# preacherwhite/Deformable-3D-Gaussians

Hardware: AMD Instinct MI355X
Metric: train iters/s (deform+raster fwd+bwd), 100k Gaussians @ 800x800 (higher is better)
Workload: dtype fp32

## Files before the change

### deformable-3d-gaussians_amd/csrc/mlp_split.hip

```cpp
#include <hip/hip_runtime.h>

#include <atomic>
#include <cassert>

#include <algorithm>
#include <cmath>
#include <cstdlib>
#include <map>
#include <mutex>
#include <type_traits>
#include <vector>

#include "dgs_common.h"
#include "mlp_shared.h"

namespace dgs {
namespace mlps {

using namespace mlpc;

typedef float f32x16 __attribute__((ext_vector_type(16)));
typedef float f32x4 __attribute__((ext_vector_type(4)));
typedef float f32x2 __attribute__((ext_vector_type(2)));
typedef _Float16 h16x8 __attribute__((ext_vector_type(8)));
// ... 78 lines not shown
}

__device__ __forceinline__ void lds_fmax(uint32_t *p, float v) {
    __hip_atomic_fetch_max(p, __float_as_uint(v), __ATOMIC_RELAXED, __HIP_MEMORY_SCOPE_WORKGROUP);
}

struct alignas(16) ScaleLDS {
    float ksc[12][4];
    float amax[2][16][4];
    float ain[2][4];
    uint32_t bsync[8][4];
    uint32_t bmax[10];
    uint32_t wstat[10];
};
constexpr int BS_XE = 0, BS_TE = 1, BS_TIN = 2, BS_TH = 3, BS_TET = 4, BS_G = 5, BS_GTE = 6;

__device__ inline float4 amax_of4(const ScaleLDS *sc, int par, int nw) {
    float4 m = make_float4(0.f, 0.f, 0.f, 0.f);
    for (int w = 0; w < nw; w++) {
        const float4 v = *reinterpret_cast<const float4 *>(sc->amax[par][w]);
        m = make_float4(fmaxf(m.x, v.x), fmaxf(m.y, v.y), fmaxf(m.z, v.z), fmaxf(m.w, v.w));
    }
    return m;
}
__device__ __forceinline__ float f4get(const float4 &v, int q) { return q == 0 ? v.x : q == 1 ? v.y : q == 2 ? v.z : v.w; }

#define MF16(a, b, c) __builtin_amdgcn_mfma_f32_16x16x32_f16((a), (b), (c), 0, 0, 0)

struct AFrag {
    h16x8 h, l;
};

__device__ inline AFrag load_a(const h16x8 *p) { return AFrag{p[0], p[64]}; }

__device__ inline AFrag load_b(const h16x8 *p, int q) { return AFrag{p[16 * q], p[BM + 16 * q]}; }

__device__ inline f32x4 zero4() { return f32x4{0.f, 0.f, 0.f, 0.f}; }

__device__ inline void mma3(const AFrag &a, const AFrag &b, f32x4 &acc, f32x4 &lo) {
    lo = MF16(a.l, b.h, lo);
    lo = MF16(a.h, b.l, lo);
    acc = MF16(a.h, b.h, acc);
}

__device__ __forceinline__ float a_inv(const h16x8 *tile_slot0) {
    return reinterpret_cast<const float *>(tile_slot0 + 128)[0];
}

#ifdef DGS_MLP_PROFILE
__device__ unsigned long long *dgs_mlps_prof;
#define DGS_STAMP(k)                                                                                   \
    do {                                                                                               \
        if (threadIdx.x == 0 && p0 == (int)blockIdx.x * BM)                                            \
            dgs_mlps_prof[blockIdx.x * 64 + (k)] = __builtin_amdgcn_s_memtime();                       \
    } while (0)
#define DGS_WSTAMP(k, L)                                                                               \
    do {                                                                                               \
        if (L == 3 && (threadIdx.x & 63) == 0 && p0 == (int)blockIdx.x * BM)                           \
            dgs_mlps_prof[blockIdx.x * 64 + (k) + (threadIdx.x >> 6)] = __builtin_amdgcn_s_memtime();  \
    } while (0)
#ifndef DGS_PROF_LAYER
#define DGS_PROF_LAYER 3
#endif
#define DGS_WSTAMP8(k, L)                                                                              \
    do {                                                                                               \
        if (L == DGS_PROF_LAYER && (threadIdx.x & 63) == 0 && p0 == (int)blockIdx.x * BM)              \
            dgs_mlps_prof[blockIdx.x * 64 + (k) + (threadIdx.x >> 6)] = __builtin_amdgcn_s_memtime();  \
    } while (0)
#else
#define DGS_WSTAMP8(k, L) \
    do {                  \
    } while (0)
#define DGS_WSTAMP(k, L) \
    do {                 \
    } while (0)
#define DGS_STAMP(k) \
    do {             \
    } while (0)
#endif

struct NoPre {
    __device__ void operator()() const {}
};

__device__ uint32_t dgs_mlps_guard_expired;

#ifdef DGS_CLOCK_STAMPS
constexpr int CLK_BLOCKS = 2048;
__device__ unsigned long long dgs_clk[3][CLK_BLOCKS][6];
struct ClkStamp {
    unsigned long long t, r;
    __device__ ClkStamp() : t(__builtin_amdgcn_s_memtime()), r(__builtin_amdgcn_s_memrealtime()) {}
    __device__ void end(int k) const {
        const unsigned long long t1 = __builtin_amdgcn_s_memtime(), r1 = __builtin_amdgcn_s_memrealtime();
        if (threadIdx.x == 0 && blockIdx.x < CLK_BLOCKS) {
            unsigned long long *p = dgs_clk[k][blockIdx.x];
            p[0] = t; p[1] = t1; p[2] = r; p[3] = r1;
            p[4] = (unsigned long long)__builtin_amdgcn_s_getreg((31 << 11) | 4) |
                   ((unsigned long long)__builtin_amdgcn_s_getreg((31 << 11) | 20) << 32);
        }
    }
};
#define CLK_BEGIN() const ClkStamp clk_
#define CLK_END(k) clk_.end(k)
#else
#define CLK_BEGIN()
#define CLK_END(k)
#endif
#ifndef DGS_SPIN_SLEEP
#define DGS_SPIN_SLEEP 1
#endif
__device__ __forceinline__ uint32_t lds_peek(const uint32_t *f) {
    return __hip_atomic_load(f, __ATOMIC_RELAXED, __HIP_MEMORY_SCOPE_WORKGROUP);
}
__device__ __forceinline__ void lds_wait_ge(const uint32_t *f, uint32_t target, uint32_t seen) {
    if (__builtin_amdgcn_readfirstlane(seen) < target) {
        int guard = 0;
#pragma clang loop unroll(disable)
        do {
            __builtin_amdgcn_s_sleep(DGS_SPIN_SLEEP);
            seen = lds_peek(f);
        } while (__builtin_amdgcn_readfirstlane(seen) < target && ++guard < (1 << 20));
        if (guard == (1 << 20) && (threadIdx.x & 63) == 0)
            __hip_atomic_fetch_add(&dgs_mlps_guard_expired, 1u, __ATOMIC_RELAXED, __HIP_MEMORY_SCOPE_AGENT);
    }
    asm volatile("" ::: "memory");
}
__device__ __forceinline__ void lds_signal(uint32_t *f, int lane) {
    asm volatile("" ::: "memory");
    if (lane == 0) __hip_atomic_fetch_add(f, 1u, __ATOMIC_RELAXED, __HIP_MEMORY_SCOPE_WORKGROUP);
}

struct NoGate {
    __device__ uint32_t peek(int) const { return 0; }
    __device__ void need(int, uint32_t) const {}
    __device__ void done(int) const {}
};

struct HGate {
    uint32_t *wr, *rd;
    int k0;
    uint32_t wt;
    bool sig;
    int lane;
    __device__ uint32_t peek(int k) const { return k < k0 ? 0xffffffffu : lds_peek(wr + (k - k0)); }
    __device__ void need(int k, uint32_t seen) const {
        if (k >= k0) lds_wait_ge(wr + (k - k0), wt, seen);
    }
    __device__ void done(int k) const {
        if (sig && k >= k0) lds_signal(rd + (k - k0), lane);
    }
};

template <int NK, int NQ_, class Pre = NoPre, class Gate = NoGate, int SKIP = (1 << 20), unsigned BND = 0u>
__device__ inline void gemm(const h16x8 *__restrict__ Aw, const h16x8 *lds, int g0, int q0, int lane,
                            f32x4 (&acc)[NQ_], float (&ib)[NQ_], const float (*ksc)[4], Pre pre = Pre(),
                            Gate gate = Gate()) {
    static_assert(NK >= 1, "empty GEMM");
    const int kq = lane >> 4, col = lane & 15;
    const h16x8 *Ap = Aw + lane;
    const int bunit = (g0 + kq) * UG + 16 * q0 + col;
    constexpr int AK = KSLOT;
    constexpr int BK = KG * UG;
    auto bofs = [](int k) { return (k + (k >= SKIP ? 1 : 0)) * BK; };
    auto kidx = [&](int k) { return (g0 >> 2) + k + (k >= SKIP ? 1 : 0); };
    auto kbase = [&](int k) {
        int u = bunit + bofs(k);
        asm volatile("" : "+v"(u));
        return lds + u;
    };
    constexpr int RING = 2;
    AFrag ring[RING];
#pragma unroll
    for (int k = 0; k < RING; k++)
        if (k < NK) ring[k] = load_a(Ap + k * AK);
    pre();
    gate.need(0, gate.peek(0));
    float cur[NQ_], nxt[NQ_];
#pragma unroll
    for (int q = 0; q < NQ_; q++) nxt[q] = cur[q] = ksc[kidx(0)][q0 + q];
    const h16x8 *Bk = kbase(0);
    AFrag b = load_b(Bk, 0);
    f32x4 lo[NQ_];
#pragma unroll
    for (int q = 0; q < NQ_; q++) lo[q] = zero4();
#pragma unroll
    for (int k = 0; k < NK; k++) {
        __builtin_amdgcn_sched_barrier(0);
        if (k > 0) gate.done(k - 1);
        if (k > 0 && k < 32 && ((BND >> k) & 1u)) {
#pragma unroll
            for (int q = 0; q < NQ_; q++) {
                acc[q] = (acc[q] + lo[q]) * (cur[q] / nxt[q]);
                lo[q] = zero4();
                cur[q] = nxt[q];
            }
        }
        const uint32_t seen = k + 1 < NK ? gate.peek(k + 1) : 0u;
#pragma unroll
        for (int q = 0; q < NQ_; q++) {
            AFrag nb;
            if (q + 1 < NQ_) nb = load_b(Bk, q + 1);
            else if (k + 1 < NK) {
                gate.need(k + 1, seen);
                if (k + 1 < 32 && ((BND >> (k + 1)) & 1u))
#pragma unroll
                    for (int q2 = 0; q2 < NQ_; q2++) nxt[q2] = ksc[kidx(k + 1)][q0 + q2];
                Bk = kbase(k + 1);
                nb = load_b(Bk, 0);
            }
            __builtin_amdgcn_sched_barrier(0);
            mma3(ring[k % RING], b, acc[q], lo[q]);
            if (q + 1 < NQ_ || k + 1 < NK) b = nb;
            __builtin_amdgcn_sched_barrier(0);
        }
        if (k + RING < NK) ring[k % RING] = load_a(Ap + (k + RING) * AK);
        __builtin_amdgcn_sched_barrier(0);
    }
    gate.done(NK - 1);
#pragma unroll
    for (int q = 0; q < NQ_; q++) {
        acc[q] += lo[q];
        ib[q] = cur[q];
    }
}

template <int NK, int NQ_, class Pre = NoPre, class Gate = NoGate, int SKIP = (1 << 20), unsigned BND = 0u>
__device__ inline void gemm2(const h16x8 *__restrict__ Aw, int astride, const h16x8 *lds, int g0, int q0, int lane,
                             f32x4 (&acc)[2][NQ_], float (&ib)[NQ_], const float (*ksc)[4], Pre pre = Pre(),
                             Gate gate = Gate()) {
    static_assert(NK >= 1, "empty GEMM");
    const int kq = lane >> 4, col = lane & 15;
    const h16x8 *Ap0 = Aw + lane, *Ap1 = Aw + astride + lane;
    const int bunit = (g0 + kq) * UG + 16 * q0 + col;
    constexpr int AK = KSLOT;
    constexpr int BK = KG * UG;
    auto bofs = [](int k) { return (k + (k >= SKIP ? 1 : 0)) * BK; };
    auto kidx = [&](int k) { return (g0 >> 2) + k + (k >= SKIP ? 1 : 0); };
    auto kbase = [&](int k) {
        int u = bunit + bofs(k);
        asm volatile("" : "+v"(u));
        return lds + u;
    };
    constexpr int RING = 2;
    AFrag ring[RING][2];
#pragma unroll
    for (int k = 0; k < RING; k++)
        if (k < NK) {
            ring[k][0] = load_a(Ap0 + k * AK);
            ring[k][1] = load_a(Ap1 + k * AK);
        }
    pre();
    gate.need(0, gate.peek(0));
    float cur[NQ_], nxt[NQ_];
#pragma unroll
    for (int q = 0; q < NQ_; q++) nxt[q] = cur[q] = ksc[kidx(0)][q0 + q];
    const h16x8 *Bk = kbase(0);
    AFrag b = load_b(Bk, 0);
    f32x4 lo[2][NQ_];
#pragma unroll
    for (int t = 0; t < 2; t++)
#pragma unroll
        for (int q = 0; q < NQ_; q++) lo[t][q] = zero4();
#pragma unroll
    for (int k = 0; k < NK; k++) {
        __builtin_amdgcn_sched_barrier(0);
        if (k > 0) gate.done(k - 1);
        if (k > 0 && k < 32 && ((BND >> k) & 1u)) {
#pragma unroll
            for (int q = 0; q < NQ_; q++) {
                const float r = cur[q] / nxt[q];
#pragma unroll
                for (int t = 0; t < 2; t++) {
                    acc[t][q] = (acc[t][q] + lo[t][q]) * r;
                    lo[t][q] = zero4();
                }
                cur[q] = nxt[q];
            }
        }
        const uint32_t seen = k + 1 < NK ? gate.peek(k + 1) : 0u;
#pragma unroll
        for (int q = 0; q < NQ_; q++) {
            AFrag nb;
            if (q + 1 < NQ_) nb = load_b(Bk, q + 1);
            else if (k + 1 < NK) {
                gate.need(k + 1, seen);
                if (k + 1 < 32 && ((BND >> (k + 1)) & 1u))
#pragma unroll
                    for (int q2 = 0; q2 < NQ_; q2++) nxt[q2] = ksc[kidx(k + 1)][q0 + q2];
                Bk = kbase(k + 1);
                nb = load_b(Bk, 0);
            }
            __builtin_amdgcn_sched_barrier(0);
            mma3(ring[k % RING][0], b, acc[0][q], lo[0][q]);
            mma3(ring[k % RING][1], b, acc[1][q], lo[1][q]);
            if (q + 1 < NQ_ || k + 1 < NK) b = nb;
            __builtin_amdgcn_sched_barrier(0);
        }
        if (k + RING < NK) {
            ring[k % RING][0] = load_a(Ap0 + (k + RING) * AK);
            ring[k % RING][1] = load_a(Ap1 + (k + RING) * AK);
        }
        __builtin_amdgcn_sched_barrier(0);
    }
    gate.done(NK - 1);
#pragma unroll
    for (int t = 0; t < 2; t++)
#pragma unroll
        for (int q = 0; q < NQ_; q++) acc[t][q] += lo[t][q];
#pragma unroll
    for (int q = 0; q < NQ_; q++) ib[q] = cur[q];
}

__device__ inline void acc_to_lds(const f32x4 &v, h16x8 *lds, int gbase, int r, int q, int lane, float S) {
    const int kq = lane >> 4, col = lane & 15;
    const Split4 s = split4(v[0], v[1], v[2], v[3], S);
    h16x4 *u = reinterpret_cast<h16x4 *>(lds + (gbase + 2 * r + (kq >> 1)) * UG + 16 * q + col) + (kq & 1);
    u[0] = s.h;
    u[2 * BM] = s.l;
}

struct Tile16 {
    __amdgpu_buffer_rsrc_t rsrc;
    int voff;
    int ns4;
#ifndef DGS_TILE_STORE_AUX
#define DGS_TILE_STORE_AUX 2
#endif
    __device__ void st(int i, int q, float v) const {
        __builtin_amdgcn_raw_buffer_store_b32(__float_as_uint(v), rsrc, voff + 64 * q, i * ns4, DGS_TILE_STORE_AUX);
    }
    template <int NQ_>
    __device__ void store(const f32x4 (&v)[NQ_], int q0 = 0) const {
#pragma unroll
        for (int q = 0; q < NQ_; q++)
#pragma unroll
            for (int i = 0; i < 4; i++) st(i, q0 + q, v[q][i]);
    }
};

__device__ inline Tile16 tile16(const float *dst, size_t Ns, int row0, int p0, int lane) {
    const float *base = dst + (size_t)row0 * Ns + p0;
    return Tile16{__builtin_amdgcn_make_buffer_rsrc(const_cast<float *>(base), 0, 0x7fffffff, 0x00020000),
                  (4 * (lane >> 4) * (int)Ns + (lane & 15)) * 4, (int)Ns * 4};
}

template <int NQ_>
__device__ inline uint32_t relu_bits(const f32x4 (&v)[NQ_]) {
    uint32_t w = 0;
#pragma unroll
    for (int q = 0; q < NQ_; q++)
#pragma unroll
        for (int i = 0; i < 4; i++) {
            uint32_t m;
            asm("v_med3_i32 %0, %1, 0, 1" : "=v"(m) : "v"(__float_as_int(v[q][i])));
            if (q == 0 && i == 0) w = m;
            else asm("v_lshl_or_b32 %0, %1, %2, %3" : "=v"(w) : "v"(m), "i"(4 * q + i), "v"(w));
        }
    return w;
}

template <int NQ_>
__device__ inline void mask_apply(f32x4 (&v)[NQ_], uint32_t bits) {
#pragma unroll
    for (int q = 0; q < NQ_; q++)
#pragma unroll
        for (int i = 0; i < 4; i++) {
            int m;
            asm("v_bfe_i32 %0, %1, %2, 1" : "=v"(m) : "v"(bits), "i"(4 * q + i));
            v[q][i] = __int_as_float(__float_as_int(v[q][i]) & m);
        }
}

__device__ inline float4 load_bias4(const float *bias, int r, int lane) {
    return *reinterpret_cast<const float4 *>(bias + 16 * r + 4 * (lane >> 4));
}

template <int NQ_>
__device__ inline void bias_relu(f32x4 (&v)[NQ_], float ia, const float (&ib)[NQ_], float4 b, bool relu) {
#pragma unroll
    for (int q = 0; q < NQ_; q++) {
        v[q] = v[q] * (ia * ib[q]) + f32x4{b.x, b.y, b.z, b.w};
        if (relu)
#pragma unroll
            for (int i = 0; i < 4; i++) v[q][i] = fmaxf(v[q][i], 0.f);
    }
}

template <int NQ_>
__device__ inline void scale_tiles(f32x4 (&v)[NQ_], float ia, const float (&ib)[NQ_]) {
#pragma unroll
    for (int q = 0; q < NQ_; q++) v[q] *= ia * ib[q];
}

template <int NQ_>
__device__ inline void zero_tiles(f32x4 (&v)[NQ_]) {
#pragma unroll
    for (int q = 0; q < NQ_; q++) v[q] = zero4();
}

__device__ __forceinline__ int queue_take(uint32_t *q) { return (int)gridDim.x + (int)atomicAdd(q, 1u); }
__device__ __forceinline__ void queue_release(uint32_t *q) {
    if (threadIdx.x == 0 && atomicAdd(q + 1, 1u) == gridDim.x - 1) {
        atomicExch(q, 0u);
        atomicExch(q + 1, 0u);
    }
}

struct FwdArgs {
    int N;
    size_t Ns;
    const float *xyz, *t;
    const h16x8 *img;
    const float *fp;
    float *out;
    float *saved;
    uint32_t *mask;
    float *tc;
    int nfull;
    int fT1, fT2, fL[8], fHd;
    int bT1, bT2, bL[8], bHd;
    int wT1, wT2;
    int w0te, w5te;
    int flags;
    uint32_t *queue;
    int nblk;
};

__device__ __forceinline__ float tile_stat(const h16x8 *tile_slot0) {
// ... 666 lines not shown
            if (lane == 0) {
                sc->amax[0][r][q] = my[q];
                sc->ksc[G_BH / 4 + (r >> 1)][q] = s.inv;
            }
            acc_to_lds(c[q], lds, G_BH, r, q, lane, s.s);
        }
        lds_signal(hwr + (r >> 1), lane);
    }
    f32x4 te5[1] = {zero4()};
#pragma unroll 1
    for (int L = 7; L >= 1; L--) {
        const uint32_t step = 8 - L;
        if (TE_ROWS && L == 5 && r < 2 * NQB) {
            const h16x8 *At = a.img + (size_t)(a.tL[5] + (F_TE / 16 + r / NQB) * 8) * KSLOT;
            float ib1[1];
            gemm<8, 1>(At, lds, G_BH, r % NQB, lane, te5, ib1, sc->ksc, NoPre(), HGate{hwr, hrd, 0, 2u * step, false, lane});
            te5[0] *= a_inv(At) * ib1[0];
        }
        const int tile0 = (L == 5) ? F_H / 16 : 0;
        uint32_t mk;
        zero_tiles(c);
        const h16x8 *Aw = a.img + (size_t)(a.tL[L] + (tile0 + r) * 8) * KSLOT;
        gemm<8, NQB>(Aw, lds, G_BH, 0, lane, c, ib, sc->ksc, trunk_pre(&mk, L - 1), HGate{hwr, hrd, 0, 2u * step, true, lane});
        scale_tiles(c, a_inv(Aw), ib);
        mask_apply(c, mk);
#ifndef DGS_DIAG_NOSAVE
        tile16(a.dz, Ns, Z_L0 + (L - 1) * 256 + 16 * r, p0, lane).store(c);
#endif
        float so[NQB], my[NQB] = {};
        chain_scales(sc, __uint_as_float(sc->wstat[L]), (step - 1) & 1, NWAVE, so);
        col_absmax(c, my);
        col_wave_max(my);
        lds_wait_ge(hrd + (r >> 1), 16u * step, lds_peek(hrd + (r >> 1)));
#pragma unroll
        for (int q = 0; q < NQB; q++) {
            const Scale s = scale_for(so[q]);
            if (lane == 0) {
                sc->amax[step & 1][r][q] = my[q];
                sc->ksc[G_BH / 4 + (r >> 1)][q] = s.inv;
            }
            acc_to_lds(c[q], lds, G_BH, r, q, lane, s.s);
        }
        lds_signal(hwr + (r >> 1), lane);
    }
    if (!TE_ROWS) return;
    if (r < 2 * NQB) {
        const int nt = r / NQB, q = r % NQB;
        f32x4 t0[1] = {zero4()};
        float ib1[1];
        const h16x8 *At = a.img + (size_t)(a.tL[0] + (F_TE / 16 + nt) * 8) * KSLOT;
        gemm<8, 1>(At, lds, G_BH, q, lane, t0, ib1, sc->ksc, NoPre(), HGate{hwr, hrd, 0, 16u, false, lane});
        te5[0] += t0[0] * (a_inv(At) * ib1[0]);
        tile16(a.dz, Ns, Z_TE + 16 * nt, p0, lane).store(te5, q);
        float tm[1] = {0.f};
        col_absmax(te5, tm);
        col_wave_max(tm);
        if (lane == 0) lds_fmax(&sc->bsync[BS_GTE][q], tm[0]);
    }
    lds_barrier();
    if (r < 2 * NQB)
        acc_to_lds(te5[0], lds, G_BG, r / NQB, r % NQB, lane, scale_for(__uint_as_float(sc->bsync[BS_GTE][r % NQB])).s);
    if (tid < 4) sc->ksc[G_BG / 4][tid] = scale_for(__uint_as_float(sc->bsync[BS_GTE][tid])).inv;
    lds_barrier();
    {
        uint32_t mk;
        zero_tiles(c);
        const h16x8 *A2 = a.img + (size_t)(a.tT2 + r) * KSLOT;
        gemm<1, NQB>(A2, lds, G_BG, 0, lane, c, ib, sc->ksc, MaskPre{&mk, mask_tile(MR_TH + r), lane});
        scale_tiles(c, a_inv(A2), ib);
        mask_apply(c, mk);
        tile16(a.dz, Ns, Z_T1 + 16 * r, p0, lane).store(c);
    }
}

struct MaskPre32x2 {
    uint32_t *mk;
    const uint32_t *word;
    int shift, lane;
    __device__ void operator()() const {
        mk[0] = word[lane] >> shift;
        mk[1] = word[64 + lane] >> shift;
    }
};
template <int NQB>
__device__ __forceinline__ void bwd_block8(const BwdArgs &a, h16x8 *lds, uint32_t *hwr, uint32_t *hrd, ScaleLDS *sc,
                                           int p0, int slot) {
    float *lf = reinterpret_cast<float *>(lds);
    float *stage = lf + G_BH * UG * 4;
    int tid = threadIdx.x;
    asm volatile("" : "+v"(tid));
    const int lane = tid & 63;
    const int w = __builtin_amdgcn_readfirstlane(tid >> 6);
    const Flags F = make_flags(a.flags);
    const size_t Ns = a.Ns;
    const uint32_t *mwords = a.mask + (size_t)slot * 2 * F.nmask;
    auto trunk_pre = [&](uint32_t *mk, int L) {
        return MaskPre32x2{mk, mwords + (size_t)(16 * (L >> 1) + 2 * w) * 64, 16 * (L & 1), lane};
    };
    if (tid < 8) {
        hwr[tid] = 0;
        hrd[tid] = 0;
    }
    stage_dout<NQB, NTHR8>(a, lds, sc, stage, p0, tid);
    f32x4 c[2][NQB];
    float ib[NQB];
    auto epilogue = [&](const h16x8 *Aw, int astride, const uint32_t (&mk)[2], int zrow, float ws, int par_in,
                        uint32_t step) {
        float my[NQB] = {};
#pragma unroll
        for (int t = 0; t < 2; t++) {
            scale_tiles(c[t], a_inv(Aw + t * astride), ib);
            mask_apply(c[t], mk[t]);
#ifndef DGS_DIAG_NOSAVE
            tile16(a.dz, Ns, zrow + 16 * (2 * w + t), p0, lane).store(c[t]);
#endif
            col_absmax(c[t], my);
        }
        float so[NQB];
        chain_scales(sc, ws, par_in, NW8, so);
        col_wave_max(my);
        if (step > 0) lds_wait_ge(hrd + w, (uint32_t)NW8 * step, lds_peek(hrd + w));
#pragma unroll
        for (int q = 0; q < NQB; q++) {
            const Scale s = scale_for(so[q]);
            if (lane == 0) {
                sc->amax[step & 1][w][q] = my[q];
                sc->ksc[G_BH / 4 + w][q] = s.inv;
            }
#pragma unroll
            for (int t = 0; t < 2; t++) acc_to_lds(c[t][q], lds, G_BH, 2 * w + t, q, lane, s.s);
        }
        lds_signal(hwr + w, lane);
    };
    {
        uint32_t mk[2];
#pragma unroll
        for (int t = 0; t < 2; t++) zero_tiles(c[t]);
        const h16x8 *Ah = a.img + (size_t)(a.tHd + 2 * w) * KSLOT;
        gemm2<1, NQB>(Ah, KSLOT, lds, G_BG, 0, lane, c, ib, sc->ksc, trunk_pre(mk, 7));
        epilogue(Ah, KSLOT, mk, Z_L0 + 7 * 256, __uint_as_float(sc->wstat[8]), -1, 0u);
    }
#pragma unroll 1
    for (int L = 7; L >= 1; L--) {
        const uint32_t step = 8 - L;
        const int tile0 = (L == 5) ? F_H / 16 : 0;
        uint32_t mk[2];
#pragma unroll
        for (int t = 0; t < 2; t++) zero_tiles(c[t]);
        const h16x8 *Aw = a.img + (size_t)(a.tL[L] + (tile0 + 2 * w) * 8) * KSLOT;
        gemm2<8, NQB>(Aw, 8 * KSLOT, lds, G_BH, 0, lane, c, ib, sc->ksc, trunk_pre(mk, L - 1),
                      HGate{hwr, hrd, 0, step, true, lane});
        epilogue(Aw, 8 * KSLOT, mk, Z_L0 + (L - 1) * 256, __uint_as_float(sc->wstat[L]), (int)((step - 1) & 1), step);
    }
}

__global__ __launch_bounds__(NTHR8) void k_bwd8(BwdArgs a) {
    __shared__ h16x8 lds[G_BWD * UG];
    __shared__ uint32_t hwr[8], hrd[8];
    __shared__ int s_next;
    __shared__ ScaleLDS sc;
    load_wstats_bwd(a, &sc);
    for (int b = blockIdx.x;;) {
        int nx = 0;
        if (a.queue && threadIdx.x == 0) nx = queue_take(a.queue);
        if (b < a.nfull) bwd_block8<NQ>(a, lds, hwr, hrd, &sc, b * BM, b);
        else bwd_block8<1>(a, lds, hwr, hrd, &sc, a.nfull * BM + (b - a.nfull) * 16, b);
        if (!a.queue) break;
        if (threadIdx.x == 0) s_next = nx;
        __syncthreads();
        b = s_next;
        if (b >= a.nblk) break;
    }
    if (a.queue) queue_release(a.queue);
}

template <bool TE_ROWS>
__global__ __launch_bounds__(NTHR) void k_bwd(BwdArgs a) {
    __shared__ h16x8 lds[G_BWD * UG];
    __shared__ uint32_t hwr[8], hrd[8];
    __shared__ int s_next;
    __shared__ ScaleLDS sc;
    load_wstats_bwd(a, &sc);
    CLK_BEGIN();
    for (int b = blockIdx.x;;) {
        int nx = 0;
        if (a.queue && threadIdx.x == 0) nx = queue_take(a.queue);
        if (b < a.nfull) bwd_block<TE_ROWS, NQ>(a, lds, hwr, hrd, &sc, b * BM, b);
        else bwd_block<TE_ROWS, 1>(a, lds, hwr, hrd, &sc, a.nfull * BM + (b - a.nfull) * 16, b);
        if (!a.queue) break;
        if (threadIdx.x == 0) s_next = nx;
        __syncthreads();
        b = s_next;
        if (b >= a.nblk) break;
    }
    if (a.queue) queue_release(a.queue);
    CLK_END(1);
}

constexpr int TG_WG = 8, TG_N = 256 / TG_WG;
struct TGradArgs {
    const float *fp;
    int w0te, w5te, wT2;
    const float *tc;
    const float *gb0, *gb5;
    float *gT0w, *gT0b, *gT2w, *gT2b;
    float *gW0, *gW5;
    int tin;
};

__global__ __launch_bounds__(1024) void k_tgrad(TGradArgs a) {
    __shared__ float S[32], th[TG_N], dz1[TG_N], Sp[32][33];
    const int j = threadIdx.x;
    const int n0 = blockIdx.x * TG_N;
    if (j < TG_N) th[j] = a.tc[TC_TH + n0 + j];
    {
        const int k = j & 31, part = j >> 5;
        float s = 0.f;
#pragma unroll
        for (int i = 0; i < 16; i++) {
            const int n = part * 16 + i;
            const float w = n < 256 ? a.fp[a.w0te + n * 32 + k] : a.fp[a.w5te + (n - 256) * 32 + k];
            const float gb = n < 256 ? a.gb0[n] : a.gb5[n - 256];
            s = fmaf(w, gb, s);
        }
        Sp[part][k] = s;
        __syncthreads();
        if (j < 32) {
            float t = 0.f;
#pragma unroll
            for (int q = 0; q < 32; q++) t += Sp[q][j];
            S[j] = t;
        }
    }
    for (int e = j; e < TG_N * 30; e += 1024) {
        const int n = n0 + e / 30, k = e % 30;
        const float te = a.tc[TC_TE + k];
        a.gW0[n * 93 + 63 + k] = a.gb0[n] * te;
        a.gW5[n * 349 + 63 + k] = a.gb5[n] * te;
    }
    __syncthreads();
    for (int e = j; e < 30 * TG_N; e += 1024) {
        const int k = e / TG_N, n = e % TG_N;
        a.gT2w[k * 256 + n0 + n] = S[k] * th[n];
    }
    if (blockIdx.x == 0 && j < 30) a.gT2b[j] = S[j];
    if (j < 4 * TG_N) {
        const int n = j >> 2, q = j & 3;
        float d = 0.f;
#pragma unroll
// ... 513 lines not shown
        (void)hipFree(d);
        return nullptr;
    }
    g_pack_units[{dev, flags}] = d;
    return d;
}

static const double kDwsShapeCost[5] = {1.0, 0.34, 0.58, 0.30, 0.41};
static WPlan split_wplan(const Flags &F, int target = 256) {
    static const bool model = env_starts("DGS_DWS_TILE_MODEL", '1');
    return make_wplan(F, target, 1.5, 4.0, model ? nullptr : kDwsShapeCost);
}


static size_t padded_points(int N) { return (size_t)div_up(N, BM) * BM; }

constexpr int TAIL_MAX_LAST = 128;
struct Blocks {
    int nfull, ntail;
};
static int cu_count() {
    static std::mutex mu;
    static std::map<int, int> cache;
    int dev = 0;
    if (hipGetDevice(&dev) != hipSuccess) return 256;
    std::lock_guard<std::mutex> lk(mu);
    auto it = cache.find(dev);
    if (it != cache.end()) return it->second;
    int v = 0;
    if (hipDeviceGetAttribute(&v, hipDeviceAttributeMultiprocessorCount, dev) != hipSuccess || v <= 0) v = 256;
    cache[dev] = v;
    return v;
}
static std::atomic<int> g_reserve_cus{-1};
static int reserved_cus() {
    int v = g_reserve_cus.load();
    if (v < 0) {
        const char *e = getenv("DGS_MLP_RESERVE_CUS");
        int want = e ? atoi(e) : 0;
        want = want < 0 ? 0 : want > 64 ? 64 : want;
        g_reserve_cus.compare_exchange_strong(v, want);
        v = g_reserve_cus.load();
    }
    return v;
}
static int mlp_cus() { return std::max(1, cu_count() - reserved_cus()); }
static Blocks block_split(int N) {
    const int nb = div_up(N, BM);
    static const bool off = env_starts("DGS_MLP_NO_TAIL", '1');
    if (off || nb == 0) return {nb, 0};
    const int ncu = mlp_cus();
    const int rounds = div_up(nb, ncu), last = nb - ncu * (rounds - 1);
    if (rounds < 2 || last > TAIL_MAX_LAST || 4 * last > ncu) return {nb, 0};
    return {nb - last, 4 * last};
}
static uint32_t *block_queue(hipStream_t stream, int kernel) {
    static const bool off = env_starts("DGS_MLP_STATIC", '1');
    if (off) return nullptr;
    static std::mutex mu;
    static std::map<std::pair<int, hipStream_t>, uint32_t *> words;
    int dev = 0;
    if (hipGetDevice(&dev) != hipSuccess) return nullptr;
    std::lock_guard<std::mutex> lk(mu);
    uint32_t *&w = words[{dev, stream}];
    if (!w) {
        if (hipMalloc(&w, 4 * sizeof(uint32_t)) != hipSuccess) {
            w = nullptr;
            return nullptr;
        }
        if (hipMemset(w, 0, 4 * sizeof(uint32_t)) != hipSuccess) return nullptr;
    }
    return w + 2 * kernel;
}
static float *timenet_scratch(hipStream_t stream) {
    static std::mutex mu;
    static std::map<std::pair<int, hipStream_t>, float *> bufs;
    int dev = 0;
    if (hipGetDevice(&dev) != hipSuccess) return nullptr;
    std::lock_guard<std::mutex> lk(mu);
    float *&b = bufs[{dev, stream}];
    if (!b && hipMalloc(&b, TC_FLOATS * sizeof(float)) != hipSuccess) b = nullptr;
    return b;
}
static int persistent_grid(int nblk, const uint32_t *queue) { return queue ? std::min(nblk, mlp_cus()) : nblk; }

static size_t mask_words(const Flags &F, size_t Ns) {
    const size_t nb = Ns / BM;
    return (size_t)F.nmask * 2 * (nb + 3 * std::min<size_t>(nb, TAIL_MAX_LAST));
}

size_t saved_floats(int flags, int N) {
    const Flags F = make_flags(flags);
    const size_t Ns = padded_points(N);
    return (size_t)F.nsaved * Ns + mask_words(F, Ns) + TC_FLOATS;
}

static int dw_mode() {
    static const int m = env_starts("DGS_MLP_SPLIT_DW", '0') ? 0 : 3;
    return m;
}
static int dw_split_once(const Flags &F, size_t Ns, const float *dz, const float *saved, float *slabs,
                         float *const *grads, hipStream_t stream);

size_t scratch_floats(int flags, int N) {
    const Flags F = make_flags(flags);
    const size_t slabs = std::max((size_t)split_wplan(F).nblocks * SLAB, mlp::dw_fp32_slab_floats(flags));
    return (size_t)F.nz * padded_points(N) + slabs;
}

int pack(int flags, const float *const *params, float *packed, hipStream_t stream) {
    const Plan P = make_plan(flags);
    if (P.nparams > PACK_MAXP) {
        set_error("dgs_deform_pack: too many parameters");
        return DGS_ERR_ARGS;
    }
    PackPtrs src{};
    for (int k = 0; k < P.nparams; k++) {
        if (!params[k]) {
            set_error("dgs_deform_pack: null parameter pointer");
            return DGS_ERR_ARGS;
        }
        src.p[k] = params[k];
    }
    const int *map = pack_map_for(P, flags);
    const int2 *units = pack_units_for(P, flags);
    if (!map || !units) {
        set_error("dgs_deform_pack: could not allocate the pack map");
        return DGS_ERR_HIP;
    }
    const int nimg = P.nslots * 512, nunits = (int)P.units.size() / 2;
    hipLaunchKernelGGL(k_pack, dim3(nunits + div_up(P.nf32, 512)), dim3(512), 0, stream, map, src, units, nunits,
                       reinterpret_cast<_Float16 *>(packed), packed + P.img_floats(), nimg, P.nf32);
    DGS_LAUNCH_CHECK("k_pack", false, stream);
    return DGS_OK;
}

static void fwd_args(const Plan &P, int flags, int N, const float *xyz, const float *t, const float *packed, float *out,
                     float *saved, FwdArgs &a, hipStream_t stream);

int forward(int flags, int N, const float *xyz, const float *t, const float *packed, float *out, float *saved,
            hipStream_t stream) {
    const Plan P = make_plan(flags);
    FwdArgs a{};
    fwd_args(P, flags, N, xyz, t, packed, out, saved, a, stream);
    const int grid = persistent_grid(a.nblk, a.queue);
    if (P.F.blender && (saved || P.F.uniform_t)) {
        if (!a.tc) {
            set_error("dgs_deform_forward: could not allocate the timenet scratch");
            return DGS_ERR_HIP;
        }
        hipLaunchKernelGGL(k_timenet, dim3(1), dim3(256), 0, stream, a);
    }
    {
        ScopedTimer tm("mlp_fwd", stream);
        const bool fold = P.F.uniform_t;
        static const bool fwd8 = !env_starts("DGS_MLP_FWD8", '0');
        if (saved && fold && fwd8)
            hipLaunchKernelGGL(k_fwd8, dim3(grid), dim3(NTHR8), 0, stream, a);
        else if (saved && fold)
            hipLaunchKernelGGL((k_fwd<true, true>), dim3(grid), dim3(NTHR), 0, stream, a);
        else if (saved)
            hipLaunchKernelGGL((k_fwd<true, false>), dim3(grid), dim3(NTHR), 0, stream, a);
        else if (fold)
            hipLaunchKernelGGL((k_fwd<false, true>), dim3(grid), dim3(NTHR), 0, stream, a);
        else
            hipLaunchKernelGGL((k_fwd<false, false>), dim3(grid), dim3(NTHR), 0, stream, a);
    }
    DGS_LAUNCH_CHECK("k_fwd", false, stream);
    return DGS_OK;
}

int pack_forward(int flags, const float *const *params, int N, const float *xyz, const float *t, float *packed,
                 float *out, float *saved, hipStream_t stream) {
    if (int rc = pack(flags, params, packed, stream)) return rc;
    return forward(flags, N, xyz, t, packed, out, saved, stream);
}

static void fwd_args(const Plan &P, int flags, int N, const float *xyz, const float *t, const float *packed, float *out,
                     float *saved, FwdArgs &a, hipStream_t stream) {
    a.N = N;
    a.Ns = padded_points(N);
    a.xyz = xyz; a.t = t; a.out = out; a.saved = saved;
    a.img = reinterpret_cast<const h16x8 *>(packed);
    a.fp = packed + P.img_floats();
    a.mask = saved ? reinterpret_cast<uint32_t *>(saved + (size_t)P.F.nsaved * a.Ns) : nullptr;
    a.fT1 = P.fT1; a.fT2 = P.fT2; a.fHd = P.fHd;
    a.bT1 = P.bT1; a.bT2 = P.bT2; a.bHd = P.bHd; a.wT1 = P.wT1; a.wT2 = P.wT2;
    a.w0te = P.w0te; a.w5te = P.w5te;
    for (int i = 0; i < 8; i++) { a.fL[i] = P.fL[i]; a.bL[i] = P.bL[i]; }
    a.flags = flags;
    const Blocks bs = block_split(N);
    a.nfull = bs.nfull;
    const int nblk = bs.nfull + bs.ntail;
    a.nblk = nblk;
    a.queue = nblk > 0 ? block_queue(stream, 0) : nullptr;
    a.tc = nullptr;
    if (P.F.blender && (saved || P.F.uniform_t))
        a.tc = saved ? saved + (size_t)P.F.nsaved * a.Ns + mask_words(P.F, a.Ns) : timenet_scratch(stream);
}

int backward(int flags, int N, const float *packed, const float *saved, const float *dout, float *scratch,
             float *const *grads, hipStream_t stream) {
    const Plan P = make_plan(flags);
    const Flags &F = P.F;
    const size_t Ns = padded_points(N);
    float *dz = scratch;
    float *slabs = scratch + (size_t)F.nz * Ns;
    BwdArgs b{};
    b.N = N; b.Ns = Ns; b.dout = dout; b.dz = dz;
    b.img = reinterpret_cast<const h16x8 *>(packed);
    b.mask = reinterpret_cast<const uint32_t *>(saved + (size_t)F.nsaved * Ns);
    b.tHd = P.tHd; b.tT2 = P.tT2;
    for (int i = 0; i < 8; i++) b.tL[i] = P.tL[i];
    b.flags = flags;
    const Blocks bs = block_split(N);
    b.nfull = bs.nfull;
    const int nblk = bs.nfull + bs.ntail;
    b.nblk = nblk;
    b.queue = nblk > 0 ? block_queue(stream, 1) : nullptr;
    const int grid = persistent_grid(nblk, b.queue);
    {
        ScopedTimer tm("mlp_bwd", stream);
        if (F.blender && !F.uniform_t)
            hipLaunchKernelGGL(k_bwd<true>, dim3(grid), dim3(NTHR), 0, stream, b);
        else
        {
            static const bool bwd8 = !env_starts("DGS_MLP_BWD8", '0');
            if (bwd8)
                hipLaunchKernelGGL(k_bwd8, dim3(grid), dim3(NTHR8), 0, stream, b);
            else
                hipLaunchKernelGGL(k_bwd<false>, dim3(grid), dim3(NTHR), 0, stream, b);
        }
    }
    DGS_LAUNCH_CHECK("k_bwd", false, stream);
    int rc;
    if (dw_mode() == 0)
        rc = mlp::dw_fp32(F, Ns, dz, saved, slabs, grads, stream);
    else
        rc = dw_split_once(F, Ns, dz, saved, slabs, grads, stream);
    if (rc != DGS_OK || !F.uniform_t) return rc;
    TGradArgs g{};
    g.fp = packed + P.img_floats();
    g.w0te = P.w0te; g.w5te = P.w5te; g.wT2 = P.wT2;
    g.tc = saved + (size_t)F.nsaved * Ns + mask_words(F, Ns);
    g.gb0 = grads[P.pLb[0]]; g.gb5 = grads[P.pLb[5]];
    g.gT0w = grads[P.pT0w]; g.gT0b = grads[P.pT0b]; g.gT2w = grads[P.pT2w]; g.gT2b = grads[P.pT2b];
    g.gW0 = grads[P.pLw[0]]; g.gW5 = grads[P.pLw[5]];
    g.tin = F.tin;
    {
        ScopedTimer tm("mlp_tgrad", stream);
        hipLaunchKernelGGL(k_tgrad, dim3(TG_WG), dim3(1024), 0, stream, g);
    }
    DGS_LAUNCH_CHECK("k_tgrad", false, stream);
    return DGS_OK;
}

static std::atomic<long long> g_dw_fallbacks{0};
static int dw_split_once(const Flags &F, size_t Ns, const float *dz, const float *saved, float *slabs,
                         float *const *grads, hipStream_t stream) {
    if ((size_t)WT * Ns * 4 >= 0x7fffffffull) {
        g_dw_fallbacks.fetch_add(1);
        return mlp::dw_fp32(F, Ns, dz, saved, slabs, grads, stream);
    }
    const WPlan W = split_wplan(F, std::max(32, 256 - reserved_cus()));
    for (int q = 0; q < W.jobs.n; q++) {
        const WJob &j = W.jobs.j[q];
        const bool ok = (j.krows == 256 && (j.nrows == 256 || j.nrows == 32)) ||
                        (j.nrows == 256 && (j.krows == 96 || j.krows == 64 || j.krows == 16));
        if (!ok) {
            set_error("dgs_deform_backward: dW job shape outside k_dws's instantiations");
            return DGS_ERR_ARGS;
        }
    }
    {
        if (int rc = ensure_dynamic_lds((const void *)k_dws, S_LDS)) return rc;
        ScopedTimer tm("mlp_dw", stream);
        hipLaunchKernelGGL(k_dws, dim3(W.nblocks), dim3(DW_THREADS), S_LDS, stream, W.jobs, Ns, dz, saved, slabs);
    }
    DGS_LAUNCH_CHECK("k_dws", false, stream);
    return launch_dw_reduce(F, W, slabs, grads, stream);
}

}
}

#ifdef DGS_MLP_PROFILE
extern "C" void dgs_mlps_set_prof(unsigned long long *p) {
    (void)hipMemcpyToSymbol(HIP_SYMBOL(dgs::mlps::dgs_mlps_prof), &p, sizeof(p));
}
#endif

using namespace dgs;

static bool exact_fp32(int flags) { return (flags & DGS_MLP_EXACT_FP32) != 0; }
static int net_flags(int flags) {
    return exact_fp32(flags) ? flags & (DGS_MLP_BLENDER | DGS_MLP_6DOF | DGS_MLP_NO_ROTSCALE)
                             : flags & (DGS_MLP_BLENDER | DGS_MLP_6DOF | DGS_MLP_NO_ROTSCALE | DGS_MLP_UNIFORM_T);
}

#ifdef DGS_CLOCK_STAMPS
extern "C" int dgs_debug_clock(int k, int n, unsigned long long *out) {
    static unsigned long long h[mlps::CLK_BLOCKS][6];
    if (k < 0 || k > 2 || n > mlps::CLK_BLOCKS) return -1;
    if (hipMemcpyFromSymbol(h, HIP_SYMBOL(dgs::mlps::dgs_clk), sizeof(h), sizeof(h) * k) != hipSuccess) return -1;
    for (int b = 0; b < n; b++)
        for (int q = 0; q < 6; q++) out[6 * b + q] = h[b][q];
    return 0;
}
#endif

extern "C" void dgs_mlp_set_reserved_cus(int k) { mlps::g_reserve_cus.store(k < 0 ? 0 : k > 64 ? 64 : k); }
extern "C" int dgs_mlp_reserved_cus(void) { return mlps::reserved_cus(); }
// ... 81 lines not shown
```

Baseline: 599.3.

## Park backward dz tiles in LDS and drain them during next layer's GEMM

In the 8-wave backward MLP kernel, each layer's dz output tiles are now parked in a per-wave LDS slice rather than stored straight to global memory. They are drained during the next layer's GEMM k-loop as one 128-bit buffer store per step, interleaved through a new Drain hook in gemm2. The aim is to take the scattered 32-bit epilogue stores off the critical path and overlap them with MFMA work. The cost is extra LDS per block, which may reduce occupancy, and more instructions inside the GEMM loop. It is on by default and can be disabled with an env var.

```diff
diff --git a/deformable-3d-gaussians_amd/csrc/mlp_split.hip b/deformable-3d-gaussians_amd/csrc/mlp_split.hip
--- a/deformable-3d-gaussians_amd/csrc/mlp_split.hip
+++ b/deformable-3d-gaussians_amd/csrc/mlp_split.hip
@@ -184,6 +184,12 @@
 struct NoPre {
     __device__ void operator()() const {}
 };
+struct NoDrain {
+    template <int NK>
+    __device__ void rd(int) const {}
+    template <int NK>
+    __device__ void st(int) const {}
+};
 
 __device__ uint32_t dgs_mlps_guard_expired;
 
@@ -327,10 +333,11 @@
     }
 }
 
-template <int NK, int NQ_, class Pre = NoPre, class Gate = NoGate, int SKIP = (1 << 20), unsigned BND = 0u>
+template <int NK, int NQ_, class Pre = NoPre, class Gate = NoGate, int SKIP = (1 << 20), unsigned BND = 0u,
+          class Dr = NoDrain>
 __device__ inline void gemm2(const h16x8 *__restrict__ Aw, int astride, const h16x8 *lds, int g0, int q0, int lane,
                              f32x4 (&acc)[2][NQ_], float (&ib)[NQ_], const float (*ksc)[4], Pre pre = Pre(),
-                             Gate gate = Gate()) {
+                             Gate gate = Gate(), Dr dr = Dr()) {
     static_assert(NK >= 1, "empty GEMM");
     const int kq = lane >> 4, col = lane & 15;
     const h16x8 *Ap0 = Aw + lane, *Ap1 = Aw + astride + lane;
@@ -368,6 +375,7 @@
     for (int k = 0; k < NK; k++) {
         __builtin_amdgcn_sched_barrier(0);
         if (k > 0) gate.done(k - 1);
+        dr.template rd<NK>(k);
         if (k > 0 && k < 32 && ((BND >> k) & 1u)) {
 #pragma unroll
             for (int q = 0; q < NQ_; q++) {
@@ -404,6 +412,8 @@
             ring[k % RING][1] = load_a(Ap1 + (k + RING) * AK);
         }
         __builtin_amdgcn_sched_barrier(0);
+        dr.template st<NK>(k);
+        __builtin_amdgcn_sched_barrier(0);
     }
     gate.done(NK - 1);
 #pragma unroll
@@ -447,6 +457,49 @@
                   (4 * (lane >> 4) * (int)Ns + (lane & 15)) * 4, (int)Ns * 4};
 }
 
+typedef uint32_t u32x4 __attribute__((ext_vector_type(4)));
+constexpr int WB_RS = 16 * NQ + 4;
+template <int NQB, int NT>
+struct WriteBehind {
+    static constexpr int RS = 16 * NQB + 4, LPR = 4 * NQB, RPS = 64 / LPR, NSH = NT * NQB, SPT = NSH / NT;
+    float *slice;
+    const float *dst;
+    int ns4;
+    int lane;
+    f32x4 v;
+    __device__ void park(int t, const f32x4 (&c)[NQB]) const {
+        float *p = slice + (16 * t + 4 * (lane >> 4)) * RS + (lane & 15);
+#pragma unroll
+        for (int q = 0; q < NQB; q++)
+#pragma unroll
+            for (int i = 0; i < 4; i++) p[i * RS + 16 * q] = c[q][i];
+    }
+    __device__ void rd(int j) {
+        v = *reinterpret_cast<const f32x4 *>(slice + (RPS * j + lane / LPR) * RS + 4 * (lane % LPR));
+    }
+    __device__ void st(int j) const {
+        const __amdgpu_buffer_rsrc_t rsrc = __builtin_amdgcn_make_buffer_rsrc(
+            const_cast<float *>(dst + (size_t)(16 * (j / SPT)) * (size_t)(ns4 >> 2)), 0, 0x7fffffff, 0x00020000);
+        __builtin_amdgcn_raw_buffer_store_b128(__builtin_bit_cast(u32x4, v), rsrc,
+                                               (lane / LPR) * ns4 + 16 * (lane % LPR), (j % SPT) * RPS * ns4,
+                                               DGS_TILE_STORE_AUX);
+    }
+};
+template <class WB>
+struct Drain {
+    WB wb;
+    template <int NK>
+    static constexpr int first(int k) { return (k * WB::NSH + NK - 1) / NK; }
+    template <int NK>
+    __device__ void rd(int k) {
+        static_assert(WB::NSH <= NK, "at most one share per k-step");
+        if (first<NK>(k) < first<NK>(k + 1)) wb.rd(first<NK>(k));
+    }
+    template <int NK>
+    __device__ void st(int k) const {
+        if (first<NK>(k) < first<NK>(k + 1)) wb.st(first<NK>(k));
+    }
+};
 template <int NQ_>
 __device__ inline uint32_t relu_bits(const f32x4 (&v)[NQ_]) {
     uint32_t w = 0;
@@ -1279,9 +1332,9 @@
         mk[1] = word[64 + lane] >> shift;
     }
 };
-template <int NQB>
+template <int NQB, bool WB>
 __device__ __forceinline__ void bwd_block8(const BwdArgs &a, h16x8 *lds, uint32_t *hwr, uint32_t *hrd, ScaleLDS *sc,
-                                           int p0, int slot) {
+                                           float *wslice, int p0, int slot) {
     float *lf = reinterpret_cast<float *>(lds);
     float *stage = lf + G_BH * UG * 4;
     int tid = threadIdx.x;
@@ -1301,18 +1354,28 @@
     stage_dout<NQB, NTHR8>(a, lds, sc, stage, p0, tid);
     f32x4 c[2][NQB];
     float ib[NQB];
+#ifndef DGS_DIAG_NOSAVE
+    constexpr bool PARK = WB;
+#else
+    constexpr bool PARK = false;
+#endif
+    using WBuf = WriteBehind<NQB, 2>;
+    WBuf wb{wslice + w * (32 * WB_RS), nullptr, (int)Ns * 4, lane, zero4()};
     auto epilogue = [&](const h16x8 *Aw, int astride, const uint32_t (&mk)[2], int zrow, float ws, int par_in,
                         uint32_t step) {
         float my[NQB] = {};
+        const bool park = PARK && step < 7;
 #pragma unroll
         for (int t = 0; t < 2; t++) {
             scale_tiles(c[t], a_inv(Aw + t * astride), ib);
             mask_apply(c[t], mk[t]);
 #ifndef DGS_DIAG_NOSAVE
-            tile16(a.dz, Ns, zrow + 16 * (2 * w + t), p0, lane).store(c[t]);
+            if (park) wb.park(t, c[t]);
+            else tile16(a.dz, Ns, zrow + 16 * (2 * w + t), p0, lane).store(c[t]);
 #endif
             col_absmax(c[t], my);
         }
+        if (park) wb.dst = a.dz + (size_t)(zrow + 32 * w) * Ns + p0;
         float so[NQB];
         chain_scales(sc, ws, par_in, NW8, so);
         col_wave_max(my);
@@ -1345,23 +1408,34 @@
 #pragma unroll
         for (int t = 0; t < 2; t++) zero_tiles(c[t]);
         const h16x8 *Aw = a.img + (size_t)(a.tL[L] + (tile0 + 2 * w) * 8) * KSLOT;
-        gemm2<8, NQB>(Aw, 8 * KSLOT, lds, G_BH, 0, lane, c, ib, sc->ksc, trunk_pre(mk, L - 1),
-                      HGate{hwr, hrd, 0, step, true, lane});
+        DGS_WSTAMP8(24, L);
+        if constexpr (PARK)
+            gemm2<8, NQB, MaskPre32x2, HGate, 1 << 20, 0u, Drain<WBuf>>(Aw, 8 * KSLOT, lds, G_BH, 0, lane, c, ib, sc->ksc,
+                                                                        trunk_pre(mk, L - 1),
+                                                                        HGate{hwr, hrd, 0, step, true, lane}, Drain<WBuf>{wb});
+        else
+            gemm2<8, NQB>(Aw, 8 * KSLOT, lds, G_BH, 0, lane, c, ib, sc->ksc, trunk_pre(mk, L - 1),
+                          HGate{hwr, hrd, 0, step, true, lane});
+        DGS_WSTAMP8(32, L);
         epilogue(Aw, 8 * KSLOT, mk, Z_L0 + (L - 1) * 256, __uint_as_float(sc->wstat[L]), (int)((step - 1) & 1), step);
-    }
-}
-
+        DGS_WSTAMP8(56, L);
+    }
+}
+
+template <bool WB>
 __global__ __launch_bounds__(NTHR8) void k_bwd8(BwdArgs a) {
     __shared__ h16x8 lds[G_BWD * UG];
     __shared__ uint32_t hwr[8], hrd[8];
     __shared__ int s_next;
     __shared__ ScaleLDS sc;
+    __shared__ f32x4 s_wb[WB ? NW8 * 32 * WB_RS / 4 : 1];
+    float *wslice = reinterpret_cast<float *>(s_wb);
     load_wstats_bwd(a, &sc);
     for (int b = blockIdx.x;;) {
         int nx = 0;
         if (a.queue && threadIdx.x == 0) nx = queue_take(a.queue);
-        if (b < a.nfull) bwd_block8<NQ>(a, lds, hwr, hrd, &sc, b * BM, b);
-        else bwd_block8<1>(a, lds, hwr, hrd, &sc, a.nfull * BM + (b - a.nfull) * 16, b);
+        if (b < a.nfull) bwd_block8<NQ, WB>(a, lds, hwr, hrd, &sc, wslice, b * BM, b);
+        else bwd_block8<1, WB>(a, lds, hwr, hrd, &sc, wslice, a.nfull * BM + (b - a.nfull) * 16, b);
         if (!a.queue) break;
         if (threadIdx.x == 0) s_next = nx;
         __syncthreads();
@@ -2041,6 +2115,10 @@
     if (!b && hipMalloc(&b, TC_FLOATS * sizeof(float)) != hipSuccess) b = nullptr;
     return b;
 }
+static bool write_behind() {
+    static const bool on = !env_starts("DGS_MLP_WRITE_BEHIND", '0');
+    return on;
+}
 static int persistent_grid(int nblk, const uint32_t *queue) { return queue ? std::min(nblk, mlp_cus()) : nblk; }
 
 static size_t mask_words(const Flags &F, size_t Ns) {
@@ -2185,8 +2263,10 @@
         else
         {
             static const bool bwd8 = !env_starts("DGS_MLP_BWD8", '0');
-            if (bwd8)
-                hipLaunchKernelGGL(k_bwd8, dim3(grid), dim3(NTHR8), 0, stream, b);
+            if (bwd8 && write_behind())
+                hipLaunchKernelGGL(k_bwd8<true>, dim3(grid), dim3(NTHR8), 0, stream, b);
+            else if (bwd8)
+                hipLaunchKernelGGL(k_bwd8<false>, dim3(grid), dim3(NTHR8), 0, stream, b);
             else
                 hipLaunchKernelGGL(k_bwd<false>, dim3(grid), dim3(NTHR), 0, stream, b);
         }
```

Result: no change. 601.8 (median of 4 runs) (+0.4%).
